# 236088/reflect-sampling-nerf

Hardware: AMD Instinct MI355X
Metric: rays/sec (train step) at 4096 rays x 128 samples, 1/2/4/8 MI355X; PSNR vs ref (higher is better)
Workload: dtype f32

## Files before the change

reflect_sampling_nerf_amd/csrc/rsn_field_kernel.h:

```cpp
#pragma once
#include "rsn_mfma.h"

#include "rsn_field_common.h"

template <int NB, bool TRAIN, int MMA>
__global__ __launch_bounds__(256) void rsn_field_kernel(const FieldJobs J) {
  constexpr bool FOLD = MMA == RSN_MMA_F32_FOLDED;
  constexpr int MODE = FOLD ? 0 : MMA;
  static_assert(!FOLD || TRAIN, "the folded bottleneck serves the exact-fp32 training kernels");
  constexpr int NBH = FOLD ? 5 : NB + 1;
  constexpr int XITS = (NB * 4 > 16) ? NB * 4 : 16;
  constexpr int WAVE_F4 = (XITS + RSN_AUX_ITS) * 64;
  constexpr int W = NB * 32;
  constexpr bool SBF = TRAIN && MODE == 3;
  __shared__ float4 smem[4 * WAVE_F4];

  const int lane = threadIdx.x & 63;
  const int wid = __builtin_amdgcn_readfirstlane(threadIdx.x >> 6);
  float4* X = smem + wid * WAVE_F4 + lane;
  float4* AUX = X + XITS * 64;
  float* Xf = reinterpret_cast<float*>(X);

  const FieldShared& P = J.s;
  const TileJobs T = tile_space<128>(J);
  const float* __restrict__ pk = P.packed;

  for (long long gtile = blockIdx.x; gtile < T.n_tiles; gtile += gridDim.x) {
    const TileAt ta = tile_at(T, gtile);
    const FieldJob& a = J.j[ta.job];
    const long long n_points = ta.n_points, tile = ta.tile;
    const long long p0 = tile * 128 + wid * 32;
    if (p0 >= n_points) continue;
    int ln = lane;
    asm volatile("" : "+v"(ln));
    const int m = ln & 31, h = ln >> 5;
    const long long p = p0 + m;
    const bool valid = p < n_points;
    const long long pc = valid ? p : n_points - 1;
    const int rows = (int)(n_points - p0 < 32 ? n_points - p0 : 32);
    constexpr bool LOOPST = TRAIN && MODE == 0;
    auto rb_epi = [&](float* base, long long elem, int row_elems) {
      return rowbuf<SBF>((TRAIN && !LOOPST) ? base : nullptr, elem, rows, row_elems, m, h);
    };
    auto rb_loop = [&](float* base, long long elem, int row_elems) {
      return rowbuf<false>(LOOPST ? base : nullptr, elem, rows, row_elems, m, h);
    };
    auto bits_at = [&](int l) -> unsigned* {
      return a.saved.relu_bits + ((((long long)l * (a.act_stride / W)) + pc) * 2 + h) * (NB / 2 > 2 ? NB / 2 : 2);
    };

    float mc[3] = {0.0f, 0.0f, 0.0f}, vc[3] = {0.0f, 0.0f, 0.0f}, vd[3] = {0.0f, 0.0f, 0.0f};
    bool has_cov = true, has_dir = true;
    float4 wbh[NBH];
    const float* __restrict__ w_bh = pk + (FOLD ? P.L.w_fold : P.L.w_bh);
    if (a.mode == RSN_MODE_EMB) {
      pre_mode<MODE, NBH>(wbh, w_bh, ln);
      has_dir = a.view_dirs != nullptr;
#pragma unroll
      for (int c = 0; c < 3; ++c) vd[c] = has_dir ? a.view_dirs[pc * 3 + c] : 0.0f;
#pragma unroll 4
      for (int it = 0; it < NB * 4; ++it)
        X[it * 64] = *reinterpret_cast<const float4*>(a.emb_in + pc * W + it * 8 + 4 * h);
    } else {
    if (a.mode == RSN_MODE_FRUSTUM || a.mode == RSN_MODE_INF) {
      has_dir = point_gaussian(a, pc, mc, vc, vd);
    } else {
      has_cov = a.cov_diag != nullptr;
      has_dir = a.view_dirs != nullptr;
#pragma unroll
      for (int c = 0; c < 3; ++c) {
        mc[c] = a.means[pc * 3 + c];
        vc[c] = has_cov ? a.cov_diag[pc * 3 + c] : 0.0f;
        vd[c] = has_dir ? a.view_dirs[pc * 3 + c] : 0.0f;
      }
    }

#pragma unroll 1
    for (int c = 0; c < 3; ++c) {
      const float x = (c == 0) ? mc[0] : (c == 1 ? mc[1] : mc[2]);
      const float v = (c == 0) ? vc[0] : (c == 1 ? vc[1] : vc[2]);
      const float sx = 6.283185307179586f * x;
#pragma unroll 2
      for (int jj = 0; jj < 8; ++jj) {
        const float f = h ? P.freqs[8 + jj] : P.freqs[jj];
        const float ang = sx * f;
        const float e = has_cov ? expf(-0.5f * (v * (f * f))) : 1.0f;
// ... 93 lines not shown
      }
    }

    {
      float sh[34];
      if (has_dir) {
        sh34_attenuated(vd[0], vd[1], vd[2], rho, sh);
      } else {
#pragma unroll
        for (int i = 0; i < 34; ++i) sh[i] = 0.0f;
      }
#pragma unroll
      for (int it = 0; it < RSN_SH_ITS; ++it) {
        float vals[4];
#pragma unroll
        for (int s = 0; s < 4; ++s) {
          const int u = it * 4 + s;
          vals[s] = (u < 17) ? (h ? sh[17 + u] : sh[u]) : 0.0f;
        }
        AUX[it * 64] = make_float4(vals[0], vals[1], vals[2], vals[3]);
        if (MODE != 0 && it == 0) AUX[5 * 64] = make_float4(0.0f, 0.0f, 0.0f, 0.0f);
        if (TRAIN && a.saved.sh && valid)
          *reinterpret_cast<float4*>(a.saved.sh + pc * RSN_K_SH_PAD + it * 8 + 4 * h) =
              make_float4(vals[0], vals[1], vals[2], vals[3]);
      }
    }

    float4 wrgb[1];
    {
      if constexpr (FOLD) {
        gemm_mode_run<MODE, 4, 4, TRAIN>(accm, wmid, pk + P.L.w_mid_sh, pk + P.L.h_mid_sh, AUX, RSN_SH_ITS, ln);
      } else {
        init_acc<4>(accm, pk + P.L.b_mid, h);
        float4 wmx[4];
        pre_mode<MODE, 4>(wmx, pk + P.L.w_mid_x, ln);
        gemm_mode_run<MODE, 4, 4, TRAIN>(accm, wmid, pk + P.L.w_mid_sh, pk + P.L.h_mid_sh, AUX, RSN_SH_ITS, ln);
        gemm_mode_run<MODE, 4, 4, TRAIN>(accm, wmx, pk + P.L.w_mid_x, pk + P.L.h_mid_x, X, NB * 4, ln, rb_loop(a.saved.bott, p0 * W, W));
      }
      pre_mode<MODE, 1>(wrgb, pk + P.L.w_rgb, ln);
      store_act<4, 4, true, SBF>(accm, X, rb_epi(a.saved.hid, p0 * 128, 128), h,
                            (TRAIN && a.saved.relu_bits && valid) ? bits_at(P.num_layers) : nullptr);
    }
    {
      f32x16 accr[1];
      init_acc<1>(accr, pk + P.L.b_rgb, h);
      gemm_mode_run<MODE, 1, 1, TRAIN>(accr, wrgb, pk + P.L.w_rgb, pk + P.L.h_rgb, X, 16, ln, rb_loop(a.saved.hid, p0 * 128, 128));
      if (h == 1 && valid) colour_out<false, TRAIN>(a, pc, accr[0][0], accr[0][1], accr[0][2], dcol, tcol);
    }

    constexpr bool SEED_BITS = TRAIN && MODE == 0;
    if (TRAIN && a.saved.normals && a.saved.relu_bits) {
      const float* __restrict__ wd = pk + P.L.v_density;
      const bool peel = SEED_BITS && P.num_layers >= 2;
      if (peel) {
        const ReluBits<NB> m7 = load_relu_bits<NB>(bits_at(P.num_layers - 1));
        const ReluBits<NB> mb = load_relu_bits<NB>(bits_at(P.num_layers - 2));
        __builtin_amdgcn_sched_barrier(0);
        f32x16 acc[NB];
        zero_acc<NB>(acc);
        if constexpr (FOLD) {
          gemm_bf16_bits<NB>(acc, pk + P.L.hT_seed, m7, ln);
        } else {
          gemm_f32_bits<NB>(acc, pk + P.L.wT_x[P.num_layers - 1], wd, m7, ln);
        }
        store_masked_bits<NB>(acc, X, mb, h);
      } else {
        const ReluBits<NB> mb = load_relu_bits<NB>(bits_at(P.num_layers - 1));
#pragma unroll
        for (int it = 0; it < NB * 4; ++it) {
          const float4 w = *reinterpret_cast<const float4*>(wd + it * 8 + 4 * h);
          const int word = mb.w[it / 8];
          const int base = ((it / 4) & 1) * 16 + 4 * (it & 3);
          X[it * 64] = make_float4(
              __uint_as_float(__float_as_uint(w.x) & bit_mask(word, base + 0)),
              __uint_as_float(__float_as_uint(w.y) & bit_mask(word, base + 1)),
              __uint_as_float(__float_as_uint(w.z) & bit_mask(word, base + 2)),
              __uint_as_float(__float_as_uint(w.w) & bit_mask(word, base + 3)));
        }
      }
      f32x16 eacc[4];
      zero_acc<4>(eacc);
#pragma unroll 1
      for (int l = P.num_layers - (peel ? 2 : 1); l >= 1; --l) {
        if (l == P.skip_layer) gemm_mode<MODE, 4, 4, TRAIN>(eacc, pk + P.L.wT_enc_skip, pk + P.L.hT_enc_skip, X, NB * 4, ln);
        const ReluBits<NB> mb = load_relu_bits<NB>(bits_at(l - 1));
        __builtin_amdgcn_sched_barrier(0);
        f32x16 acc[NB];
        zero_acc<NB>(acc);
        gemm_mode<MODE, NB, NB, TRAIN>(acc, pk + P.L.wT_x[l], pk + P.L.hT_x[l], X, NB * 4, ln);
        store_masked_bits<NB>(acc, X, mb, h);
      }
      gemm_mode<MODE, 4, 4, TRAIN>(eacc, pk + P.L.wT_enc0, pk + P.L.hT_enc0, X, NB * 4, ln);
      store_act<4, 4, false>(eacc, X);
      float nrm[3];
#pragma unroll 1
      for (int c = 0; c < 3; ++c) {
        const float x = (c == 0) ? mc[0] : (c == 1 ? mc[1] : mc[2]);
        const float v = (c == 0) ? vc[0] : (c == 1 ? vc[1] : vc[2]);
        const float sx = 6.283185307179586f * x;
        float part = 0.0f;
#pragma unroll 2
        for (int jj = 0; jj < 8; ++jj) {
          const float f = h ? P.freqs[8 + jj] : P.freqs[jj];
          const float ang = sx * f;
          const float e = has_cov ? expf(-0.5f * (v * (f * f))) : 1.0f;
          const int u = c * 8 + jj;
          const float gs = Xf[(u >> 2) * 256 + (u & 3)];
          const float gc = Xf[((u + 24) >> 2) * 256 + ((u + 24) & 3)];
          part += (gs * (e * cos_big(ang)) + gc * (e * cos_big(ang + 1.5707963267948966f))) * f;
        }
        part *= 6.283185307179586f;
        if (h == 0) part += Xf[12 * 256 + c];
        const float tot = part + __shfl_xor(part, 32, 64);
        if (c == 0) nrm[0] = tot; else if (c == 1) nrm[1] = tot; else nrm[2] = tot;
      }
      if (h == 0 && valid) {
        const float len = fmaxf(sqrtf(nrm[0] * nrm[0] + nrm[1] * nrm[1] + nrm[2] * nrm[2]), 1e-12f);
        a.saved.normals[pc * 3 + 0] = -(nrm[0] / len);
        a.saved.normals[pc * 3 + 1] = -(nrm[1] / len);
        a.saved.normals[pc * 3 + 2] = -(nrm[2] / len);
      }
    }
  }
}
```

reflect_sampling_nerf_amd/csrc/rsn_mfma.h:

```cpp
#pragma once
#include "rsn_common.h"

typedef float f32x16 __attribute__((ext_vector_type(16)));

#define RSN_MODE_FRUSTUM 0
#define RSN_MODE_INF 1
#define RSN_MODE_GAUSS 2
#define RSN_MODE_EMB 3

__device__ __forceinline__ float softplus_f(float x) { return x > 20.0f ? x : log1pf(expf(x)); }
__device__ __forceinline__ float sigmoid_f(float x) { return 1.0f / (1.0f + expf(-x)); }

__device__ __forceinline__ float sincos_big(float a, int quad) {
  const float q = rintf(a * 0.63661977236758134308f);
  float r = __builtin_fmaf(-q, 1.5707963705062866f, a);
  r = __builtin_fmaf(-q, -4.371138828673793e-08f, r);
  r = __builtin_fmaf(-q, -1.7151245100058819e-15f, r);
  const int n = (int)q + quad;
  const float s = r * r;
  const float ps = r + r * s * (-1.6666654611e-1f + s * (8.3321608736e-3f + s * (-1.9515295891e-4f)));
  const float pc =
      1.0f + s * (-0.5f + s * (4.166664568298827e-2f + s * (-1.388731625493765e-3f + s * 2.443315711809948e-5f)));
  const float v = (n & 1) ? pc : ps;
  return (n & 2) ? -v : v;
// ... 218 lines not shown
  for (; it + 1 < n_it; it += 2) {
    load_w<NBO, NBT>(wb, wp, it + 1);
    bb = xl[(it + 1) * 64];
    mma4<NBO>(acc, wa, ba);
    if (sv_on(save)) sv_put_it(save, it, ba);
    interleave_loads<NBO>();
    __builtin_amdgcn_sched_barrier(0);
    {
      const int in = (it + 2 < n_it) ? it + 2 : n_it - 1;
      load_w<NBO, NBT>(wa, wp, in);
      ba = xl[in * 64];
    }
    mma4<NBO>(acc, wb, bb);
    if (sv_on(save)) sv_put_it(save, it + 1, bb);
    interleave_loads<NBO>();
    __builtin_amdgcn_sched_barrier(0);
  }
  if (it < n_it) {
    mma4<NBO>(acc, wa, ba);
    if (sv_on(save)) sv_put_it(save, it, ba);
  }
}

template <int NBO, int NBT = NBO, bool PF2 = false, class SV = const float*>
__device__ __forceinline__ void gemm(f32x16 (&acc)[NBO], const float* __restrict__ wseg, const float4* xl, int n_it,
                                     int lane, SV save = nullptr) {
  float4 wa[NBO];
  pre_w<NBO, NBT>(wa, wseg, lane);
  if (PF2) gemm_run2<NBO, NBT>(acc, wa, wseg, xl, n_it, lane, save); else gemm_run<NBO, NBT>(acc, wa, wseg, xl, n_it, lane, save);
}

template <int NBO>
__device__ __forceinline__ void init_acc(f32x16 (&acc)[NBO], const float* __restrict__ bias, int h) {
#pragma unroll
  for (int nb = 0; nb < NBO; ++nb)
#pragma unroll
    for (int q = 0; q < 4; ++q) {
      const float4 bv = *reinterpret_cast<const float4*>(bias + nb * 32 + 8 * q + 4 * h);
      acc[nb][4 * q + 0] = bv.x;
      acc[nb][4 * q + 1] = bv.y;
      acc[nb][4 * q + 2] = bv.z;
      acc[nb][4 * q + 3] = bv.w;
    }
}

typedef __bf16 bf16x8 __attribute__((ext_vector_type(8)));

struct BSplit {
  bf16x8 s1, s2, s3;
};

template <int NSPLIT>
__device__ __forceinline__ BSplit split8(const float4 lo, const float4 hi) {
  const float x[8] = {lo.x, lo.y, lo.z, lo.w, hi.x, hi.y, hi.z, hi.w};
  BSplit o;
#pragma unroll
  for (int e = 0; e < 8; ++e) {
    const __bf16 b1 = (__bf16)x[e];
    const float r1 = x[e] - (float)b1;
    const __bf16 b2 = (NSPLIT >= 2) ? (__bf16)r1 : (__bf16)0.0f;
    o.s1[e] = b1;
    o.s2[e] = b2;
    if (NSPLIT == 3) {
      const float r2 = r1 - (float)b2;
      o.s3[e] = (__bf16)r2;
    } else {
      o.s3[e] = (__bf16)0.0f;
    }
  }
  return o;
}

template <int NH, int NSPLIT>
__device__ __forceinline__ void load_w16(bf16x8 (&w)[NH][3], const WBuf& wp, int kk, int nbo, int nb0) {
#pragma unroll
  for (int t = 0; t < NH; ++t)
#pragma unroll
    for (int sp = 0; sp < NSPLIT; ++sp) {
      const u32x4 v = __builtin_amdgcn_raw_buffer_load_b128(wp.r, wp.voff, (unsigned)(((kk * nbo + nb0 + t) * 3 + sp) * 1024), 0);
      w[t][sp] = __builtin_bit_cast(bf16x8, v);
    }
}

template <int NBO, int NH, int NB0, int NSPLIT>
__device__ __forceinline__ void mma16(f32x16 (&acc)[NBO], const bf16x8 (&w)[NH][3], const BSplit& b) {
#pragma unroll
  for (int t = 0; t < NH; ++t) {
    f32x16 c = acc[NB0 + t];
    if (NSPLIT == 3) {
      c = __builtin_amdgcn_mfma_f32_32x32x16_bf16(w[t][2], b.s1, c, 0, 0, 0);
      c = __builtin_amdgcn_mfma_f32_32x32x16_bf16(w[t][1], b.s2, c, 0, 0, 0);
      c = __builtin_amdgcn_mfma_f32_32x32x16_bf16(w[t][0], b.s3, c, 0, 0, 0);
    }
    if (NSPLIT >= 2) {
      c = __builtin_amdgcn_mfma_f32_32x32x16_bf16(w[t][1], b.s1, c, 0, 0, 0);
      c = __builtin_amdgcn_mfma_f32_32x32x16_bf16(w[t][0], b.s2, c, 0, 0, 0);
    }
    c = __builtin_amdgcn_mfma_f32_32x32x16_bf16(w[t][0], b.s1, c, 0, 0, 0);
    acc[NB0 + t] = c;
  }
}

template <int NBO, int NSPLIT>
__device__ __forceinline__ void gemm_bf16(f32x16 (&acc)[NBO], const float* __restrict__ wseg, const float4* xl,
                                          int n_k16, int lane) {
  constexpr int H0 = (NBO + 1) / 2, H1 = NBO - H0;
  constexpr int PER = (NSPLIT == 3 ? 6 : (NSPLIT == 2 ? 3 : 1));
  const WBuf wp = wbuf_make(wseg, lane);
  bf16x8 wa[H0][3], wb[H1 > 0 ? H1 : 1][3];
  load_w16<H0, NSPLIT>(wa, wp, 0, NBO, 0);
  BSplit bc = split8<NSPLIT>(xl[0], xl[64]);
  const int k1 = n_k16 > 1 ? 1 : 0;
  float4 xlo = xl[(2 * k1) * 64], xhi = xl[(2 * k1 + 1) * 64];
#pragma unroll 1
  for (int kk = 0; kk < n_k16; ++kk) {
    if (H1 > 0) load_w16<(H1 > 0 ? H1 : 1), NSPLIT>(wb, wp, kk, NBO, H0);
    __builtin_amdgcn_sched_barrier(0);
    const BSplit bn = split8<NSPLIT>(xlo, xhi);
    mma16<NBO, H0, 0, NSPLIT>(acc, wa, bc);
#pragma unroll
    for (int g = 0; g < H0 * PER; ++g) {
      __builtin_amdgcn_sched_group_barrier(0x008, 1, 0);
      __builtin_amdgcn_sched_group_barrier(0x002, 2, 0);
    }
    __builtin_amdgcn_sched_barrier(0);
    const int kn = (kk + 1 < n_k16) ? kk + 1 : kk;
    const int k2 = (kk + 2 < n_k16) ? kk + 2 : kn;
    load_w16<H0, NSPLIT>(wa, wp, kn, NBO, 0);
    xlo = xl[(2 * k2) * 64];
    xhi = xl[(2 * k2 + 1) * 64];
    __builtin_amdgcn_sched_barrier(0);
    if (H1 > 0) mma16<NBO, (H1 > 0 ? H1 : 1), (H1 > 0 ? H0 : 0), NSPLIT>(acc, wb, bc);
    __builtin_amdgcn_sched_barrier(0);
    bc = bn;
  }
}

template <int MODE, int NBO, int NBT = NBO, bool PF2 = false, class SV = const float*>
__device__ __forceinline__ void gemm_mode(f32x16 (&acc)[NBO], const float* __restrict__ w32, const float* __restrict__ w16,
                                          const float4* xl, int n_it, int lane, SV save = nullptr) {
  static_assert(MODE == 0 || NBT == NBO, "the split-bf16 loops own every output block of their segment");
  if (MODE == 0) {
    gemm<NBO, NBT, PF2>(acc, w32, xl, n_it, lane, save);
  } else {
    gemm_bf16<NBO, (MODE == 1 ? 3 : (MODE == 2 ? 2 : 1))>(acc, w16, xl, (n_it + 1) / 2, lane);
  }
}

template <int MODE, int NBO, int NBT = NBO>
__device__ __forceinline__ void pre_mode(float4 (&wa)[NBO], const float* __restrict__ w32, int lane) {
  if (MODE == 0) pre_w<NBO, NBT>(wa, w32, lane);
}

template <int MODE, int NBO, int NBT = NBO, bool PF2 = false, class SV = const float*>
__device__ __forceinline__ void gemm_mode_run(f32x16 (&acc)[NBO], float4 (&wa)[NBO], const float* __restrict__ w32,
                                              const float* __restrict__ w16, const float4* xl, int n_it, int lane,
                                              SV save = nullptr) {
  static_assert(MODE == 0 || NBT == NBO, "the split-bf16 loops own every output block of their segment");
  if (MODE == 0) {
    if (PF2) gemm_run2<NBO, NBT>(acc, wa, w32, xl, n_it, lane, save); else gemm_run<NBO, NBT>(acc, wa, w32, xl, n_it, lane, save);
  } else {
    gemm_bf16<NBO, (MODE == 1 ? 3 : (MODE == 2 ? 2 : 1))>(acc, w16, xl, (n_it + 1) / 2, lane);
  }
}

template <int NBO>
__device__ __forceinline__ void zero_acc(f32x16 (&acc)[NBO]) {
#pragma unroll
  for (int nb = 0; nb < NBO; ++nb)
#pragma unroll
    for (int r = 0; r < 16; ++r) acc[nb][r] = 0.0f;
}

__device__ __forceinline__ unsigned relu_bits16(const f32x16& a) {
  unsigned b = 0u;
#pragma unroll
  for (int r = 0; r < 16; ++r) {
    const unsigned lo = __float_as_uint(relu_f(a[r]));
    unsigned bit;
    if (r == 0) {
      asm("v_min_u32 %0, %1, 1" : "=v"(bit) : "v"(lo));
      b = bit;
    } else {
      unsigned nb;
      asm("v_min_u32 %0, %2, 1\n\tv_lshl_or_b32 %1, %0, %3, %4" : "=&v"(bit), "=v"(nb) : "v"(lo), "n"(r), "v"(b));
      b = nb;
    }
  }
  return b;
}

template <int Q>
__device__ __forceinline__ unsigned relu_bits4q(unsigned b, const float4 v) {
  const unsigned lo[4] = {__float_as_uint(v.x), __float_as_uint(v.y), __float_as_uint(v.z), __float_as_uint(v.w)};
#pragma unroll
  for (int t = 0; t < 4; ++t) {
    unsigned bit, nb;
    if (Q == 0 && t == 0) {
      asm("v_min_u32 %0, %1, 1" : "=v"(bit) : "v"(lo[t]));
      b = bit;
    } else if (t == 0) {
      asm("v_min_u32 %0, %2, 1\n\tv_lshl_or_b32 %1, %0, %3, %4" : "=&v"(bit), "=v"(nb) : "v"(lo[t]), "n"(4 * Q), "v"(b));
      b = nb;
    } else if (t == 1) {
      asm("v_min_u32 %0, %2, 1\n\tv_lshl_or_b32 %1, %0, %3, %4" : "=&v"(bit), "=v"(nb) : "v"(lo[t]), "n"(4 * Q + 1), "v"(b));
      b = nb;
    } else if (t == 2) {
      asm("v_min_u32 %0, %2, 1\n\tv_lshl_or_b32 %1, %0, %3, %4" : "=&v"(bit), "=v"(nb) : "v"(lo[t]), "n"(4 * Q + 2), "v"(b));
      b = nb;
    } else {
      asm("v_min_u32 %0, %2, 1\n\tv_lshl_or_b32 %1, %0, %3, %4" : "=&v"(bit), "=v"(nb) : "v"(lo[t]), "n"(4 * Q + 3), "v"(b));
      b = nb;
    }
  }
  return b;
// ... 83 lines not shown
#pragma unroll 1
  for (int kk = 0; kk < NK; ++kk) {
    load_w16<NH, 3>(wb, wp, kk, NBO, NH);
    __builtin_amdgcn_sched_barrier(0);
    const int kn = (kk + 1 < NK) ? kk + 1 : kk;
    const bf16x8 bn = bits_bf16x8(mw, kn);
    mma16_bits<NBO, NH>(acc, wa, bc, 0);
#pragma unroll
    for (int g = 0; g < NH * 3; ++g) {
      __builtin_amdgcn_sched_group_barrier(0x008, 1, 0);
      __builtin_amdgcn_sched_group_barrier(0x002, 2, 0);
    }
    __builtin_amdgcn_sched_barrier(0);
    load_w16<NH, 3>(wa, wp, kn, NBO, 0);
    __builtin_amdgcn_sched_barrier(0);
    mma16_bits<NBO, NH>(acc, wb, bc, NH);
    __builtin_amdgcn_sched_barrier(0);
    bc = bn;
  }
}

template <int NBO, int NH>
__device__ __forceinline__ void load_w32_pair(float4 (&f)[NH][2], const WBuf& b, int kk, int nb0) {
#pragma unroll
  for (int t = 0; t < NH; ++t)
#pragma unroll
    for (int j = 0; j < 2; ++j) {
      const u32x4 v = __builtin_amdgcn_raw_buffer_load_b128(b.r, b.voff + (unsigned)(nb0 + t) * 1024u, (unsigned)(2 * kk + j) * (NBO * 1024u), 0);
      f[t][j] = make_float4(__uint_as_float(v.x), __uint_as_float(v.y), __uint_as_float(v.z), __uint_as_float(v.w));
    }
}

template <int NBO, int NH>
__device__ __forceinline__ void mma16_bits_f32(f32x16 (&acc)[NBO], const float4 (&f)[NH][2], const float4 dlo, const float4 dhi,
                                               const bf16x8 b, int nb0) {
#pragma unroll
  for (int t = 0; t < NH; ++t) {
    const float v[8] = {rsn_seed_product(f[t][0].x, dlo.x), rsn_seed_product(f[t][0].y, dlo.y), rsn_seed_product(f[t][0].z, dlo.z),
                        rsn_seed_product(f[t][0].w, dlo.w), rsn_seed_product(f[t][1].x, dhi.x), rsn_seed_product(f[t][1].y, dhi.y),
                        rsn_seed_product(f[t][1].z, dhi.z), rsn_seed_product(f[t][1].w, dhi.w)};
    bf16x8 s1, s2, s3;
#pragma unroll
    for (int e = 0; e < 8; ++e) {
      const __bf16 b1 = (__bf16)v[e];
      const float r1 = v[e] - (float)b1;
      const __bf16 b2 = (__bf16)r1;
      const float r2 = r1 - (float)b2;
      s1[e] = b1; s2[e] = b2; s3[e] = (__bf16)r2;
    }
    f32x16 c = acc[nb0 + t];
    c = __builtin_amdgcn_mfma_f32_32x32x16_bf16(s3, b, c, 0, 0, 0);
    c = __builtin_amdgcn_mfma_f32_32x32x16_bf16(s2, b, c, 0, 0, 0);
    c = __builtin_amdgcn_mfma_f32_32x32x16_bf16(s1, b, c, 0, 0, 0);
    acc[nb0 + t] = c;
  }
}

template <int NBO>
__device__ __forceinline__ void gemm_f32_bits(f32x16 (&acc)[NBO], const float* __restrict__ w32seg, const float* __restrict__ wd,
                                              const ReluBits<NBO>& m, int lane) {
  static_assert(NBO % 2 == 0, "two fragment buffers of NBO / 2 blocks");
  constexpr int NH = NBO / 2, NK = 2 * NBO;
  const WBuf wp = wbuf_make(w32seg, lane);
  const float* __restrict__ wdl = wd + 4 * (lane >> 5);
  float4 fa[NH][2], fb[NH][2];
  load_w32_pair<NBO, NH>(fa, wp, 0, 0);
  const SeedWords mw = seed_words<NBO>(m);
  float4 dlo = *reinterpret_cast<const float4*>(wdl), dhi = *reinterpret_cast<const float4*>(wdl + 8);
#pragma unroll 1
  for (int kk = 0; kk < NK; ++kk) {
    load_w32_pair<NBO, NH>(fb, wp, kk, NH);
    const int kn = (kk + 1 < NK) ? kk + 1 : kk;
    const float4 nlo = *reinterpret_cast<const float4*>(wdl + 16 * kn), nhi = *reinterpret_cast<const float4*>(wdl + 16 * kn + 8);
    const bf16x8 bc = bits_bf16x8(mw, kk);
    mma16_bits_f32<NBO, NH>(acc, fa, dlo, dhi, bc, 0);
    __builtin_amdgcn_sched_barrier(0);
    load_w32_pair<NBO, NH>(fa, wp, kn, 0);
    mma16_bits_f32<NBO, NH>(acc, fb, dlo, dhi, bc, NH);
    __builtin_amdgcn_sched_barrier(0);
    dlo = nlo; dhi = nhi;
  }
}

__device__ __forceinline__ unsigned bit_mask(int word, int pos) {
  unsigned m;
  asm("v_bfe_i32 %0, %1, %2, 1" : "=v"(m) : "v"(word), "n"(pos));
  return m;
}

template <int NBO, bool SBF = false, class SV = float*>
__device__ __forceinline__ void store_masked_bits(const f32x16 (&acc)[NBO], float4* xl, const ReluBits<NBO>& m, int h,
                                                  SV save = nullptr) {
#pragma unroll
  for (int nb = 0; nb < NBO; ++nb)
#pragma unroll
    for (int q = 0; q < 4; ++q) {
      const int word = m.w[nb / 2];
      const int base = (nb & 1) * 16 + 4 * q;
      float4 v;
      v.x = __uint_as_float(__float_as_uint(acc[nb][4 * q + 0]) & bit_mask(word, base + 0));
      v.y = __uint_as_float(__float_as_uint(acc[nb][4 * q + 1]) & bit_mask(word, base + 1));
      v.z = __uint_as_float(__float_as_uint(acc[nb][4 * q + 2]) & bit_mask(word, base + 2));
      v.w = __uint_as_float(__float_as_uint(acc[nb][4 * q + 3]) & bit_mask(word, base + 3));
      xl[(nb * 4 + q) * 64] = v;
      if (sv_on(save)) sv_put<SBF>(save, nb, q, h, v);
    }
}

template <int NBO, int NBS, bool RELU, bool SBF = false, class SV = float*>
__device__ __forceinline__ void store_act(const f32x16 (&acc)[NBO], float4* xl, SV save = nullptr, int h = 0,
                                          unsigned* bits = nullptr) {
  unsigned bw[NBS / 2 > 0 ? NBS / 2 : 1];
#pragma unroll
  for (int nb = 0; nb < NBS; ++nb) {
    unsigned b16 = 0u;
#pragma unroll
    for (int q = 0; q < 4; ++q) {
      float4 v = make_float4(acc[nb][4 * q + 0], acc[nb][4 * q + 1], acc[nb][4 * q + 2], acc[nb][4 * q + 3]);
      if (RELU) {
        v.x = relu_f(v.x);
        v.y = relu_f(v.y);
        v.z = relu_f(v.z);
        v.w = relu_f(v.w);
        b16 = relu_bits4(b16, v, q);
      }
      xl[(nb * 4 + q) * 64] = v;
      if (sv_on(save)) sv_put<SBF>(save, nb, q, h, v);
    }
    if (RELU) {
      if (nb & 1) bw[nb / 2] |= b16 << 16; else bw[nb / 2] = b16;
    }
  }
  if (RELU && bits) {
    if (NBS >= 8) {
#pragma unroll
      for (int w4 = 0; w4 < NBS / 8; ++w4)
        *reinterpret_cast<uint4*>(bits + w4 * 4) = make_uint4(bw[w4 * 4], bw[w4 * 4 + 1], bw[w4 * 4 + 2], bw[w4 * 4 + 3]);
    } else {
#pragma unroll
      for (int w = 0; w < NBS / 2; ++w) bits[w] = bw[w];
    }
  }
}

template <int NBO, bool RELU, bool SBF = false, class SV = float*>
__device__ __forceinline__ void store_act_init(f32x16 (&acc)[NBO], float4* xl, SV save, int h,
                                               const float* __restrict__ bias, unsigned* bits = nullptr) {
  unsigned bw[NBO / 2 > 0 ? NBO / 2 : 1];
#pragma unroll
  for (int nb = 0; nb < NBO; ++nb) {
    unsigned b16 = 0u;
#pragma unroll
    for (int q = 0; q < 4; ++q) {
      float4 v = make_float4(acc[nb][4 * q + 0], acc[nb][4 * q + 1], acc[nb][4 * q + 2], acc[nb][4 * q + 3]);
      if (RELU) {
        v.x = relu_f(v.x);
        v.y = relu_f(v.y);
        v.z = relu_f(v.z);
        v.w = relu_f(v.w);
        b16 = relu_bits4(b16, v, q);
      }
      xl[(nb * 4 + q) * 64] = v;
      if (sv_on(save)) sv_put<SBF>(save, nb, q, h, v);
      const float4 bv = *reinterpret_cast<const float4*>(bias + nb * 32 + 8 * q + 4 * h);
      acc[nb][4 * q + 0] = bv.x;
      acc[nb][4 * q + 1] = bv.y;
// ... 64 lines not shown
```

reflect_sampling_nerf_amd/csrc/rsn_pack.hip:

```cpp
#include <stdarg.h>
#include <stdlib.h>
#include <string.h>

#include <string>
#include <vector>

#include "rsn_common.h"

static thread_local std::string g_last_error;

void rsn_set_error(const char* fmt, ...) {
  char buf[1024];
  va_list ap;
  va_start(ap, fmt);
  vsnprintf(buf, sizeof(buf), fmt, ap);
  va_end(ap);
  g_last_error = buf;
}

extern "C" const char* rsn_last_error(void) { return g_last_error.c_str(); }

int rsn_device_cus() {
  static int cache[64] = {0};
  int dev = 0;
// ... 458 lines not shown
    rows_from(*j, 128, enc_slot_to_column); cols_natural(*j, W, 0);
  }
  j = gemm(p->bottleneck_w, W, L.wT_bh, NB * 4, NB, 1);
  rows_natural(*j, W); cols_natural(*j, W, 0);
  j = gemm(nullptr, 0, L.wT_bh + (size_t)(NB * 4) * NB * 256, 4, NB, 3);
  heads_src(*j, 0, heads_w, W); rows_natural(*j, W); cols_headsT(*j, false);
  j = gemm(p->mid_w, mid_in, L.wT_mid_x, NBM * 4, NB, 1);
  rows_natural(*j, W, RSN_SH_DIM); cols_natural(*j, MW, 0);
  j = gemm(p->rgb_w, MW, L.wT_rgb, 4, NBM, 1);
  rows_natural(*j, MW);
  for (int c = 0; c < 3; ++c) j->col[4 + c] = (int16_t)c;
  rows_natural(*bias(p->density_w, L.v_density, WP), W);

  if (L.q_stream != 0) {
    int frag = 0;
    auto ring = [&](const float* w, int ld, int ks, int nbo16, int transpose = 0) {
      PackJob* q = gemm(w, ld, L.q_stream + (size_t)frag * 256 * L.q_pf, ks, nbo16, transpose);
      q->layout = L.q_pf == 3 ? 2 : 1;
      frag += ks * nbo16;
      return q;
    };
    for (int l = 0; l < n_layers; ++l) {
      if (l >= 1) {
        j = ring(p->trunk_w[l], in_f(l), 8, 16);
        rows_perm16(*j, WP, W); cols_natural(*j, W, x_off(l));
      }
      if (l == 0 || l == skip) {
        j = ring(p->trunk_w[l], in_f(l), 4, 16);
        rows_perm16(*j, WP, W); cols_slots(*j, 128, enc16_slot_to_column);
      }
    }
    j = ring(nullptr, W, 8, 2);
    heads_src(*j, 1, heads_w, W); heads_rows(*j, 0); cols_natural(*j, W, 0);
    j = ring(p->bottleneck_w, W, 8, 16);
    rows_perm16(*j, WP, W); cols_natural(*j, W, 0);
    j = ring(p->mid_w, mid_in, 2, 8);
    rows_perm16(*j, MW, MW); cols_slots(*j, 64, sh16_slot_to_column);
    j = ring(p->mid_w, mid_in, 8, 8);
    rows_perm16(*j, MW, MW); cols_natural(*j, W, RSN_SH_DIM);
    j = ring(p->rgb_w, MW, 4, 4);
    rows_rgb(*j); cols_natural(*j, MW, 0);
    RSN_REQUIRE(frag * L.q_pf == L.q_groups * 16, RSN_ERR_INVALID_ARGUMENT, "16x32 stream: %d fragments, layout says %d groups",
                frag, L.q_groups);
    j = ring(p->rgb_w, MW, 2, 8, 1);
    rows_perm16(*j, MW, MW);
    for (int c = 0; c < 3; ++c) j->col[8 + c] = (int16_t)c;
    j = ring(p->mid_w, mid_in, 4, 16, 1);
    rows_perm16(*j, WP, W, RSN_SH_DIM); cols_natural(*j, MW, 0);
    j = ring(p->bottleneck_w, W, 8, 16, 1);
    rows_perm16(*j, WP, W); cols_natural(*j, W, 0);
    j = ring(nullptr, 0, 1, 16, 3);
    heads_src(*j, 0, heads_w, W); rows_perm16(*j, WP, W); cols_headsT(*j, true);
    for (int l = n_layers - 1; l >= 0; --l) {
      if (l == 0 || l == skip) {
        j = ring(p->trunk_w[l], in_f(l), 8, 8, 1);
        rows_from(*j, 128, [](int n) { return enc16_slot_to_column(perm16_row_to_feature(n)); }); cols_natural(*j, W, 0);
      }
      if (l >= 1) {
        j = ring(p->trunk_w[l], in_f(l), 8, 16, 1);
        rows_perm16(*j, WP, W, x_off(l)); cols_natural(*j, W, 0);
      }
    }
    RSN_REQUIRE(frag * L.q_pf == L.t_g_end * 16, RSN_ERR_INVALID_ARGUMENT, "transposed 16x32 stream: %d fragments, layout says %d groups",
                frag, L.t_g_end);
  }

  if (d->mma_mode == RSN_MMA_F32_FOLDED) {
    const float* wc = packed + L.fold_wc;
    j = gemm(wc, W, L.w_fold, NB * 4, NBM + 1);
    heads_src(*j, 1, heads_w, W); rows_natural(*j, MW); heads_rows(*j, MW); cols_natural(*j, W, 0);
    j = bias(packed + L.fold_bc, L.b_fold, MW + 32);
    heads_src(*j, 1, heads_b, 0); rows_natural(*j, MW); heads_rows(*j, MW);
    j = gemm(wc, W, L.wT_fold, NBM * 4, NB, 1);
    rows_natural(*j, W); cols_natural(*j, MW, 0);
    j = gemm(nullptr, 0, L.wT_fold + (size_t)(NBM * 4) * NB * 256, 4, NB, 3);
    heads_src(*j, 0, heads_w, W); rows_natural(*j, W); cols_headsT(*j, false);
  }

  auto split = [&](size_t src, int n_it, int nbo, size_t dst, size_t kscale = 0) {
    splits.push_back(SplitSeg{(unsigned)src, (unsigned)dst, (short)n_it, (short)nbo, 0, (unsigned)kscale});
  };
  if (d->mma_mode == RSN_MMA_F32 || d->mma_mode == RSN_MMA_F32_FOLDED) {
    if (L.hT_seed != 0) split(L.wT_x[n_layers - 1], NB * 4, NB, L.hT_seed, L.v_density);
    return RSN_OK;
  }
  split(L.w_enc0, RSN_ENC_ITS, NB, L.h_enc0);
  for (int l = 1; l < n_layers; ++l) {
    split(L.w_x[l], NB * 4, NB, L.h_x[l]);
    split(L.wT_x[l], NB * 4, NB, L.hT_x[l]);
  }
  if (skip >= 1) {
    split(L.w_enc_skip, RSN_ENC_ITS, NB, L.h_enc_skip);
    split(L.wT_enc_skip, NB * 4, 4, L.hT_enc_skip);
  }
  split(L.wT_enc0, NB * 4, 4, L.hT_enc0);
  split(L.w_bh, NB * 4, NB + 1, L.h_bh);
  split(L.wT_bh, NB * 4 + 4, NB, L.hT_bh);
  split(L.w_mid_sh, RSN_SH_ITS, NBM, L.h_mid_sh);
  split(L.w_mid_x, NB * 4, NBM, L.h_mid_x);
  split(L.wT_mid_x, NBM * 4, NB, L.hT_mid_x);
  split(L.w_rgb, NBM * 4, 1, L.h_rgb);
  split(L.wT_rgb, 4, NBM, L.hT_rgb);
  return RSN_OK;
}

thread_local std::vector<PackJob> t_jobs;
thread_local std::vector<SplitSeg> t_splits;

int validate_and_build(const rsn_field_desc* d, const rsn_field_params* p, float* packed, size_t packed_bytes) {
  RsnPackedLayout L;
  const int rc = rsn_compute_layout(d, &L);
  if (rc != RSN_OK) return rc;
  RSN_REQUIRE(p != nullptr && packed != nullptr, RSN_ERR_INVALID_ARGUMENT, "params/packed is NULL");
  RSN_REQUIRE(packed_bytes >= L.total * sizeof(float), RSN_ERR_WORKSPACE,
              "packed buffer too small: %zu < %zu bytes", packed_bytes, L.total * sizeof(float));
  t_jobs.clear(); t_splits.clear();
  return build_jobs(d, p, packed, L, t_jobs, t_splits);
}

}

static int launch_fold(const rsn_field_desc* d, const rsn_field_params* p, float* packed, hipStream_t st) {
  if (d->mma_mode != RSN_MMA_F32_FOLDED) return RSN_OK;
  RsnPackedLayout L;
  RSN_TRY(rsn_compute_layout(d, &L));
  const int w = d->param_width > 0 ? d->param_width : d->width, n = d->mid_width * w + d->mid_width;
  hipLaunchKernelGGL(rsn_fold_kernel, dim3((unsigned)((n + 255) / 256)), dim3(256), 0, st, p->mid_w, p->mid_b, p->bottleneck_w,
                     p->bottleneck_b, w, d->mid_width, packed + L.fold_wc, packed + L.fold_bc);
  RSN_HIP(hipGetLastError());
  return RSN_OK;
}

extern "C" int rsn_pack_weights(const rsn_field_desc* d, const rsn_field_params* p, float* packed,
                                size_t packed_bytes, void* stream) {
  const int rc = validate_and_build(d, p, packed, packed_bytes);
  if (rc != RSN_OK) return rc;
  hipStream_t st = (hipStream_t)stream;
  RSN_TRY(launch_fold(d, p, packed, st));
  for (const PackJob& j : t_jobs) {
    hipLaunchKernelGGL(rsn_pack_kernel, dim3((unsigned)job_blocks(j)), dim3(256), 0, st, j);
    RSN_HIP(hipGetLastError());
  }
  for (const SplitSeg& s : t_splits) {
    hipLaunchKernelGGL(rsn_pack_split_kernel, dim3((unsigned)split_blocks(s)), dim3(256), 0, st, packed + s.src, (int)s.n_it,
                       (int)s.nbo, packed + s.dst, s.kscale ? packed + s.kscale : nullptr);
    RSN_HIP(hipGetLastError());
  }
  return RSN_OK;
}

extern "C" size_t rsn_pack_table_bytes(void) { return sizeof(PackTable); }

extern "C" int rsn_pack_weights_table(const rsn_field_desc* d, const rsn_field_params* p, float* packed,
                                      size_t packed_bytes, void* table, size_t table_bytes, int32_t rebuild_table,
                                      void* stream) {
  RSN_REQUIRE(table != nullptr && table_bytes >= sizeof(PackTable), RSN_ERR_WORKSPACE,
              "job table buffer too small: %zu < %zu bytes", table_bytes, sizeof(PackTable));
  const int rc = validate_and_build(d, p, packed, packed_bytes);
  if (rc != RSN_OK) return rc;
  RSN_REQUIRE((int)t_jobs.size() <= PACK_MAX_JOBS && (int)t_splits.size() <= SPLIT_MAX_SEGS, RSN_ERR_UNSUPPORTED,
              "%zu pack jobs / %zu split segments exceed the table", t_jobs.size(), t_splits.size());
  hipStream_t st = (hipStream_t)stream;
  static thread_local PackTable host_table;
  const int n_jobs = (int)t_jobs.size();
  int blocks = 0;
  for (int i = 0; i < n_jobs; ++i) {
// ... 27 lines not shown
```

Before: 92420.

## Emulate fp32 backward sweep GEMMs with nine-product bf16 split MFMA

Adds a sweep_gemm dispatcher so that the backward density sweep, when seed bits are used, runs its layer GEMMs as a 3-way bf16 split with all nine cross products. Weights come either pre-split by the packer (the folded mode now packs split copies of the transposed layer weights) or split on the fly from fp32. The aim is to swap the exact-fp32 MFMA path for bf16 MFMAs, which have higher throughput, while keeping accuracy close to fp32. The cost is nine MFMAs per block plus extra split VALU work and, in folded mode, extra packed weight memory.

After: 93580, median of 6. +1.3%, better.

```diff
diff --git a/reflect_sampling_nerf_amd/csrc/rsn_field_kernel.h b/reflect_sampling_nerf_amd/csrc/rsn_field_kernel.h
--- a/reflect_sampling_nerf_amd/csrc/rsn_field_kernel.h
+++ b/reflect_sampling_nerf_amd/csrc/rsn_field_kernel.h
@@ -2,6 +2,16 @@
 #include "rsn_mfma.h"
 
 #include "rsn_field_common.h"
+
+template <bool X9, bool PACKED, int MODE, int NBO>
+__device__ __forceinline__ void sweep_gemm(f32x16 (&acc)[NBO], const float* __restrict__ w32, const float* __restrict__ w16,
+                                           const float4* xl, int n_it, int lane) {
+  if constexpr (X9) {
+    if constexpr (PACKED) gemm_bf16<NBO, 3, true>(acc, w16, xl, n_it / 2, lane); else gemm_f32_x9<NBO>(acc, w32, xl, n_it / 2, lane);
+  } else {
+    gemm_mode<MODE, NBO, NBO, true>(acc, w32, w16, xl, n_it, lane);
+  }
+}
 
 template <int NB, bool TRAIN, int MMA>
 __global__ __launch_bounds__(256) void rsn_field_kernel(const FieldJobs J) {
@@ -261,15 +271,15 @@
       zero_acc<4>(eacc);
 #pragma unroll 1
       for (int l = P.num_layers - (peel ? 2 : 1); l >= 1; --l) {
-        if (l == P.skip_layer) gemm_mode<MODE, 4, 4, TRAIN>(eacc, pk + P.L.wT_enc_skip, pk + P.L.hT_enc_skip, X, NB * 4, ln);
+        if (l == P.skip_layer) sweep_gemm<SEED_BITS, FOLD, MODE, 4>(eacc, pk + P.L.wT_enc_skip, pk + P.L.hT_enc_skip, X, NB * 4, ln);
         const ReluBits<NB> mb = load_relu_bits<NB>(bits_at(l - 1));
         __builtin_amdgcn_sched_barrier(0);
         f32x16 acc[NB];
         zero_acc<NB>(acc);
-        gemm_mode<MODE, NB, NB, TRAIN>(acc, pk + P.L.wT_x[l], pk + P.L.hT_x[l], X, NB * 4, ln);
+        sweep_gemm<SEED_BITS, FOLD, MODE, NB>(acc, pk + P.L.wT_x[l], pk + P.L.hT_x[l], X, NB * 4, ln);
         store_masked_bits<NB>(acc, X, mb, h);
       }
-      gemm_mode<MODE, 4, 4, TRAIN>(eacc, pk + P.L.wT_enc0, pk + P.L.hT_enc0, X, NB * 4, ln);
+      sweep_gemm<SEED_BITS, FOLD, MODE, 4>(eacc, pk + P.L.wT_enc0, pk + P.L.hT_enc0, X, NB * 4, ln);
       store_act<4, 4, false>(eacc, X);
       float nrm[3];
 #pragma unroll 1
diff --git a/reflect_sampling_nerf_amd/csrc/rsn_mfma.h b/reflect_sampling_nerf_amd/csrc/rsn_mfma.h
--- a/reflect_sampling_nerf_amd/csrc/rsn_mfma.h
+++ b/reflect_sampling_nerf_amd/csrc/rsn_mfma.h
@@ -324,11 +324,17 @@
     }
 }
 
-template <int NBO, int NH, int NB0, int NSPLIT>
+template <int NBO, int NH, int NB0, int NSPLIT, bool FULL = false>
 __device__ __forceinline__ void mma16(f32x16 (&acc)[NBO], const bf16x8 (&w)[NH][3], const BSplit& b) {
+  static_assert(!FULL || NSPLIT == 3, "the full product is over three pieces a side");
 #pragma unroll
   for (int t = 0; t < NH; ++t) {
     f32x16 c = acc[NB0 + t];
+    if (FULL) {
+      c = __builtin_amdgcn_mfma_f32_32x32x16_bf16(w[t][2], b.s3, c, 0, 0, 0);
+      c = __builtin_amdgcn_mfma_f32_32x32x16_bf16(w[t][2], b.s2, c, 0, 0, 0);
+      c = __builtin_amdgcn_mfma_f32_32x32x16_bf16(w[t][1], b.s3, c, 0, 0, 0);
+    }
     if (NSPLIT == 3) {
       c = __builtin_amdgcn_mfma_f32_32x32x16_bf16(w[t][2], b.s1, c, 0, 0, 0);
       c = __builtin_amdgcn_mfma_f32_32x32x16_bf16(w[t][1], b.s2, c, 0, 0, 0);
@@ -343,11 +349,11 @@
   }
 }
 
-template <int NBO, int NSPLIT>
+template <int NBO, int NSPLIT, bool FULL = false>
 __device__ __forceinline__ void gemm_bf16(f32x16 (&acc)[NBO], const float* __restrict__ wseg, const float4* xl,
                                           int n_k16, int lane) {
   constexpr int H0 = (NBO + 1) / 2, H1 = NBO - H0;
-  constexpr int PER = (NSPLIT == 3 ? 6 : (NSPLIT == 2 ? 3 : 1));
+  constexpr int PER = FULL ? 9 : (NSPLIT == 3 ? 6 : (NSPLIT == 2 ? 3 : 1));
   const WBuf wp = wbuf_make(wseg, lane);
   bf16x8 wa[H0][3], wb[H1 > 0 ? H1 : 1][3];
   load_w16<H0, NSPLIT>(wa, wp, 0, NBO, 0);
@@ -359,7 +365,7 @@
     if (H1 > 0) load_w16<(H1 > 0 ? H1 : 1), NSPLIT>(wb, wp, kk, NBO, H0);
     __builtin_amdgcn_sched_barrier(0);
     const BSplit bn = split8<NSPLIT>(xlo, xhi);
-    mma16<NBO, H0, 0, NSPLIT>(acc, wa, bc);
+    mma16<NBO, H0, 0, NSPLIT, FULL>(acc, wa, bc);
 #pragma unroll
     for (int g = 0; g < H0 * PER; ++g) {
       __builtin_amdgcn_sched_group_barrier(0x008, 1, 0);
@@ -372,7 +378,7 @@
     xlo = xl[(2 * k2) * 64];
     xhi = xl[(2 * k2 + 1) * 64];
     __builtin_amdgcn_sched_barrier(0);
-    if (H1 > 0) mma16<NBO, (H1 > 0 ? H1 : 1), (H1 > 0 ? H0 : 0), NSPLIT>(acc, wb, bc);
+    if (H1 > 0) mma16<NBO, (H1 > 0 ? H1 : 1), (H1 > 0 ? H0 : 0), NSPLIT, FULL>(acc, wb, bc);
     __builtin_amdgcn_sched_barrier(0);
     bc = bn;
   }
@@ -622,6 +628,67 @@
   }
 }
 
+__device__ __forceinline__ f32x16 x9_block(f32x16 c, const BSplit& w, const BSplit& b) {
+  c = __builtin_amdgcn_mfma_f32_32x32x16_bf16(w.s3, b.s3, c, 0, 0, 0);
+  c = __builtin_amdgcn_mfma_f32_32x32x16_bf16(w.s3, b.s2, c, 0, 0, 0);
+  c = __builtin_amdgcn_mfma_f32_32x32x16_bf16(w.s2, b.s3, c, 0, 0, 0);
+  c = __builtin_amdgcn_mfma_f32_32x32x16_bf16(w.s3, b.s1, c, 0, 0, 0);
+  c = __builtin_amdgcn_mfma_f32_32x32x16_bf16(w.s2, b.s2, c, 0, 0, 0);
+  c = __builtin_amdgcn_mfma_f32_32x32x16_bf16(w.s1, b.s3, c, 0, 0, 0);
+  c = __builtin_amdgcn_mfma_f32_32x32x16_bf16(w.s2, b.s1, c, 0, 0, 0);
+  c = __builtin_amdgcn_mfma_f32_32x32x16_bf16(w.s1, b.s2, c, 0, 0, 0);
+  c = __builtin_amdgcn_mfma_f32_32x32x16_bf16(w.s1, b.s1, c, 0, 0, 0);
+  return c;
+}
+
+template <int NBO>
+__device__ __forceinline__ void gemm_f32_x9(f32x16 (&acc)[NBO], const float* __restrict__ w32seg, const float4* xl, int n_k16,
+                                            int lane) {
+  static_assert(NBO % 2 == 0, "two fragment buffers of NBO / 2 blocks");
+  constexpr int NH = NBO / 2;
+  const WBuf wp = wbuf_make(w32seg, lane);
+  float4 fa[NH][2], fb[NH][2];
+  load_w32_pair<NBO, NH>(fa, wp, 0, 0);
+  load_w32_pair<NBO, NH>(fb, wp, 0, NH);
+  BSplit bc = split8<3>(xl[0], xl[64]);
+  const int k1 = n_k16 > 1 ? 1 : 0;
+  float4 xlo = xl[(2 * k1) * 64], xhi = xl[(2 * k1 + 1) * 64];
+  BSplit w = split8<3>(fa[0][0], fa[0][1]);
+  BSplit bn = bc;
+#pragma unroll 1
+  for (int kk = 0; kk < n_k16; ++kk) {
+    const int kn = (kk + 1 < n_k16) ? kk + 1 : kk;
+    const int k2 = (kk + 2 < n_k16) ? kk + 2 : kn;
+#pragma unroll
+    for (int b = 0; b < NBO; ++b) {
+      BSplit wn;
+      if (b + 1 < NH) wn = split8<3>(fa[b + 1][0], fa[b + 1][1]);
+      else if (b + 1 < NBO) wn = split8<3>(fb[b + 1 - NH][0], fb[b + 1 - NH][1]);
+      else wn = split8<3>(fa[0][0], fa[0][1]);
+      if (b == NH - 1) load_w32_pair<NBO, NH>(fa, wp, kn, 0);
+      if (b == NBO - 1) {
+        load_w32_pair<NBO, NH>(fb, wp, kn, NH);
+        bn = split8<3>(xlo, xhi);
+        xlo = xl[(2 * k2) * 64];
+        xhi = xl[(2 * k2 + 1) * 64];
+      }
+      acc[b] = x9_block(acc[b], w, bc);
+      const bool loads = b == NH - 1 || b == NBO - 1;
+#pragma unroll
+      for (int g = 0; g < 9; ++g) {
+        __builtin_amdgcn_sched_group_barrier(0x008, 1, 0);
+        if (loads && g < 2 * NH) __builtin_amdgcn_sched_group_barrier(0x020, 1, 0);
+        if (b == NBO - 1) __builtin_amdgcn_sched_group_barrier(0x002, 8, 0);
+        else __builtin_amdgcn_sched_group_barrier(0x002, 5, 0);
+      }
+      if (b == NBO - 1) __builtin_amdgcn_sched_group_barrier(0x100, 2, 0);
+      __builtin_amdgcn_sched_barrier(0);
+      w = wn;
+    }
+    bc = bn;
+  }
+}
+
 __device__ __forceinline__ unsigned bit_mask(int word, int pos) {
   unsigned m;
   asm("v_bfe_i32 %0, %1, %2, 1" : "=v"(m) : "v"(word), "n"(pos));
diff --git a/reflect_sampling_nerf_amd/csrc/rsn_pack.hip b/reflect_sampling_nerf_amd/csrc/rsn_pack.hip
--- a/reflect_sampling_nerf_amd/csrc/rsn_pack.hip
+++ b/reflect_sampling_nerf_amd/csrc/rsn_pack.hip
@@ -564,6 +564,11 @@
   };
   if (d->mma_mode == RSN_MMA_F32 || d->mma_mode == RSN_MMA_F32_FOLDED) {
     if (L.hT_seed != 0) split(L.wT_x[n_layers - 1], NB * 4, NB, L.hT_seed, L.v_density);
+    if (d->mma_mode == RSN_MMA_F32_FOLDED) {
+      for (int l = 1; l + 1 < n_layers; ++l) split(L.wT_x[l], NB * 4, NB, L.hT_x[l]);
+      if (skip >= 1) split(L.wT_enc_skip, NB * 4, 4, L.hT_enc_skip);
+      split(L.wT_enc0, NB * 4, 4, L.hT_enc0);
+    }
     return RSN_OK;
   }
   split(L.w_enc0, RSN_ENC_ITS, NB, L.h_enc0);
```
